# erhant/halo2-vectordb

Measured on AMD Instinct MI355X. Metric: constraints/sec, proving hot path (witness+layout+commit MSM+NTT), kmeans k=16 circuit, higher is better.
Workload: dtype u32x8 (BN254 Fr/Fq, 254-bit Montgomery)

## Files before the change

### halo2_vectordb_amd/_lib.py

```python
import ctypes
import os
import subprocess

_HERE = os.path.dirname(os.path.abspath(__file__))
LIB_PATH = os.path.join(_HERE, "libvdb_hip.so")
CSRC = os.path.join(_HERE, "csrc")


class VdbError(RuntimeError):
    def __init__(self, code, msg):
        super().__init__(f"vdb error {code}: {msg}")
        self.code = code


def build(force=False, jobs=8):
    cmd = ["make", "-C", CSRC, f"-j{jobs}"]
    if force:
        cmd.append("-B")
    subprocess.check_call(cmd)
    return LIB_PATH


_lib = None

# ... 51 lines not shown
    "vdb_ann_index_apply_dev": [_P, _P, _P, _P, _P, _SZ, _SZ, _SZ, _U32, _P, _P, _P, _P, _SZ, _P, _P, _P, _P, _P],
    "vdb_wit_ann_delete_size": [_SZ, _SZ, _SZ, _SZ, _P, _P, _P, _P, _P],
    "vdb_wit_ann_delete": [_P, _P, _SZ, _SZ, _SZ, _SZ, _P, _SZ, _P, _P, _P],
    "vdb_wit_ann_delete_dev": [_P, _P, _SZ, _SZ, _SZ, _SZ, _P, _SZ, _P, _P, _P],
    "vdb_ann_index_remove_size": [_P, _SZ, _SZ, _P, _SZ, _P, _P, _P],
    "vdb_ann_index_remove_dev": [_P, _P, _P, _P, _SZ, _SZ, _SZ, _P, _P, _SZ, _P, _P, _P, _P, _P],
    "vdb_wit_ann_audit_size": [_I, _U32, _U32, _SZ, _SZ, _SZ, _P, _P, _P],
    "vdb_wit_ann_audit": [_I, _U32, _U32, _P, _P, _P, _SZ, _SZ, _SZ, _SZ, _P, _P, _P, _P, _P],
    "vdb_wit_ann_audit_dev": [_I, _U32, _U32, _P, _P, _P, _P, _P, _SZ, _SZ, _SZ, _SZ, _P, _P, _P, _P, _P],
    "vdb_wit_ann_mean_size": [_U32, _U32, _SZ, _SZ, _SZ, _P, _P, _P],
    "vdb_wit_ann_mean": [_U32, _U32, _P, _P, _P, _SZ, _SZ, _SZ, _SZ, _P, _P, _P, _P, _P],
    "vdb_wit_ann_mean_dev": [_U32, _U32, _P, _P, _P, _P, _P, _SZ, _SZ, _SZ, _SZ, _P, _P, _P, _P, _P],
    "vdb_ann_cluster_means_dev": [_U32, _U32, _P, _P, _SZ, _SZ, _SZ, _P],
    "vdb_ann_cluster_means": [_U32, _U32, _P, _P, _SZ, _SZ, _SZ, _P],
    "vdb_wit_nearest_batch_size": [_I, _U32, _U32, _SZ, _SZ, _SZ, _P, _P],
    "vdb_wit_nearest_batch": [_I, _U32, _U32, _P, _P, _SZ, _SZ, _SZ, _P, _P, _P, _P, _P],
    "vdb_wit_nearest_batch_dev": [_I, _U32, _U32, _P, _P, _SZ, _SZ, _SZ, _P, _P, _P, _P, _P],
    "vdb_wit_nearest_topk_size": [_I, _U32, _U32, _SZ, _SZ, _SZ, _SZ, _P, _P],
    "vdb_wit_nearest_topk": [_I, _U32, _U32, _P, _P, _SZ, _SZ, _SZ, _SZ, _P, _P, _P, _P, _P],
    "vdb_wit_nearest_topk_dev": [_I, _U32, _U32, _P, _P, _SZ, _SZ, _SZ, _SZ, _P, _P, _P, _P, _P],
    "vdb_nearest_values": [_U32, _U32, _I, _P, _P, _SZ, _SZ, _SZ, _P, _P],
    "vdb_nearest_values_dev": [_U32, _U32, _I, _P, _P, _SZ, _SZ, _SZ, _P, _P],
    "vdb_layout_plan": [_P, _U64, _U32, _U32, _P, _U64, _P], "vdb_layout_plan_dev": [_P, _U64, _U32, _U32, _P, _U64, _P],
    "vdb_layout_columns": [_P, _U64, _P, _U64, _P, _U64, _U32, _U32, _P, _P, _U64],
    "vdb_layout_columns_dev": [_P, _U64, _P, _U64, _U32, _P, _P, _U32],
    "vdb_layout_lookup_dev": [_P, _U64, _U32, _U32, _P, _U64, _P, _U32],
    "vdb_layout_columns_range_dev": [_P, _U64, _P, _U64, _U32, _U64, _U64, _P, _P, _U32],
    "vdb_layout_lookup_range_dev": [_P, _U64, _U32, _U32, _U64, _U64, _P, _P, _U32], "vdb_wit_set_window": [_U64, _U64, _U64, _U64],
    "vdb_g1_sum": [_P, _SZ, _SZ, _P], "vdb_srs_load": [_U32, _P, _P, _P], "vdb_srs_load_window": [_U32, _P, _P, _U32, _P], "vdb_srs_setup_unsafe": [_U32, _P, _P, _P], "vdb_srs_free": [_P], "vdb_srs_info": [_P, _P, _P, _P],
    "vdb_msm": [_P, _I, _P, _SZ, _P], "vdb_msm_batch": [_P, _I, _P, _SZ, _SZ, _P], "vdb_msm_batch_dev": [_P, _I, _P, _SZ, _SZ, _P],
    "vdb_msm_batch_masked_dev": [_P, _I, _P, _SZ, _SZ, _P, _P, _P], "vdb_layout_const_mask_dev": [_P, _U64, _P, _U64, _U32, _P],
    "vdb_mask_select_dev": [_P, _P, _U64, _I, _P],
    "vdb_msm_count_entries_dev": [_P, _P, _SZ, _SZ, _P, _P],
    "vdb_msm_batch_masked_dev_begin": [_P, _I, _P, _SZ, _SZ, _P, _P], "vdb_msm_batch_end": [_P, _SZ],
    "vdb_grand_product_dev": [_P, _P, _SZ, _SZ, _P], "vdb_eval_polys_dev": [_P, _SZ, _SZ, _P, _P], "vdb_extended_to_coeff_dev": [_P, _SZ, _U32, _U32],
    "vdb_gate_eval_dev": [_P, _P, _SZ, _U32, _U32, _P, _P], "vdb_permutation_mapping_pack_dev": [_P, _SZ, _U32, _P], "vdb_permutation_sigma_packed_dev": [_P, _SZ, _SZ, _U32, _P, _P],
    "vdb_eval_polys_dev_out": [_P, _SZ, _SZ, _P, _P], "vdb_transcript_flush": [_P],
    "vdb_gate_eval_sub_dev": [_P, _U32, _P, _SZ, _U32, _U32, _P, _P], "vdb_divide_by_vanishing_dev": [_P, _U32, _U32],
    "vdb_layout_selectors_dev": [_P, _U64, _P, _U64, _U32, _P],
    "vdb_lookup_permute_dev": [_P, _P, _SZ, _SZ, _SZ, _U32, _P, _P],
    "vdb_lookup_product_dev": [_P, _P, _P, _P, _SZ, _SZ, _SZ, _P, _P, _P], "vdb_fr_delta": [_P],
    "vdb_permutation_sigma_dev": [_P, _SZ, _U32, _P, _P],
    "vdb_transcript_new": [_U32, _U32, _U32, _P], "vdb_transcript_free": [_P], "vdb_transcript_set_sign_bit": [_P, _U32], "vdb_transcript_common_scalar": [_P, _P], "vdb_transcript_common_point": [_P, _P],
    "vdb_transcript_write_points": [_P, _P, _SZ], "vdb_transcript_write_scalars": [_P, _P, _SZ], "vdb_transcript_common_points": [_P, _P, _SZ], "vdb_transcript_common_scalars": [_P, _P, _SZ],
    "vdb_transcript_write_scalar": [_P, _P], "vdb_transcript_write_point": [_P, _P], "vdb_transcript_squeeze": [_P, _P],
    "vdb_transcript_proof_len": [_P, _P], "vdb_transcript_proof_bytes": [_P, _P, _SZ],
    "vdb_scratch_release": [], "vdb_mem_info": [_P, _P], "vdb_scratch_held": [_P], "vdb_msm_set_scratch_cap": [_SZ], "vdb_alloc_stats": [_P, _P, _P, _I],
    "vdb_permutation_mapping_dev": [_P, _U64, _U64, _P, _U64, _U32, _P, _U64, _U64, _U64, _P, _U64, _P],
    "vdb_permutation_mapping_ws_dev": [_P, _U64, _U64, _P, _U64, _U32, _P, _U64, _U64, _U64, _P, _U64, _P, _P, _SZ],
    "vdb_gather_fr_dev": [_P, _P, _SZ, _P], "vdb_copymap_init_dev": [_U64, _U64, _P, _P, _P, _P],
    "vdb_copymap_place_dev": [_P, _P, _P, _U64, _P, _U64, _P, _P, _P, _U64, _U64, _U64, _U64, _P, _P, _P, _P],
    "vdb_copymap_finish_dev": [_P, _P, _U64, _P, _U64, _P, _P, _P], "vdb_mock_check_instances_dev": [_P, _U64, _P, _P, _U64, _P],
    "vdb_fill_rows_dev": [_P, _SZ, _SZ, _SZ, _P],
    "vdb_poly_axpy_dev": [_P, _P, _P, _SZ], "vdb_poly_scale_dev": [_P, _P, _SZ],
    "vdb_poly_lincomb_dev": [_P, _SZ, _SZ, _P, _P], "vdb_kate_div_dev": [_P, _SZ, _SZ, _P, _P, _P],
    "vdb_permutation_eval_dev": [_P, _P, _P, _SZ, _SZ, _U32, _U32, _SZ, _P, _P, _P, _P, _P, _P, _P, _P],
    "vdb_permutation_eval_range_dev": [_P, _P, _P, _SZ, _SZ, _U32, _U32, _SZ, _P, _P, _P, _P, _P, _P, _P, _P, _SZ, _SZ],
    "vdb_coeff_to_cosets_dev": [_P, _P, _SZ, _U32, _U32, _P], "vdb_cosets_to_coeff_dev": [_P, _P, _U32, _U32],
    "vdb_gate_eval_cosets_dev": [_P, _U32, _P, _SZ, _U32, _U32, _P, _P],
    "vdb_lookup_eval_cosets_dev": [_P, _P, _P, _P, _P, _SZ, _U32, _U32, _P, _P, _P, _P, _P, _P, _P],
    "vdb_permutation_eval_parts_cosets_dev": [_P, _SZ, _P, _P, _SZ, _P, _P, _SZ, _SZ, _U32, _U32, _SZ, _P, _P, _P, _P, _P, _P, _P, _P, _I, _SZ, _SZ, _SZ, _SZ],
    "vdb_lookup_eval_dev": [_P, _P, _P, _P, _P, _SZ, _U32, _U32, _P, _P, _P, _P, _P, _P, _P],
    "vdb_permutation_product_dev": [_P, _P, _SZ, _U32, _SZ, _SZ, _P, _P, _P, _P],
    "vdb_permutation_product_range_dev": [_P, _P, _SZ, _SZ, _U32, _SZ, _SZ, _P, _P, _P, _P], "vdb_permutation_chain_dev": [_P, _SZ, _U32, _SZ],
    "vdb_permutation_eval_parts_dev": [_P, _SZ, _P, _P, _SZ, _P, _P, _SZ, _SZ, _U32, _U32, _SZ, _P, _P, _P, _P, _P, _P, _P, _P, _I, _SZ, _SZ, _SZ, _SZ],
    "vdb_colsrc_build_dev": [_P, _U64, _P, _U64, _U32, _U64, _U64, _P, _U32, _P],
# ... 46 lines not shown
```

### halo2_vectordb_amd/csrc/msm.hip

```cpp
#include "common.hpp"
#include "ec.hpp"
#include "ec_l9.hpp"
#include "limb9.hpp"

struct vdb_srs {
  uint32_t k;
  size_t n;
  uint32_t c, W, B;
  vdb::Affine* table[2];
  int device;
};
#define VDB_SRS_HERE(srs) VDB_ARG((srs)->device == vdb::ctx().device, "this srs handle was loaded on another device (vdb_set_device)")

namespace vdb {

#define MSM_SORT_THREADS 1024
#define MSM_LCAP_MIN 32
#define MSM_LCAP_MAX 256

struct MsmRange {
  uint32_t col, bucket, start, len, seg0, pad;
};
struct MsmSegInfo {
  uint32_t idx, len;
};

__global__ __launch_bounds__(256) void k_srs_table(const Affine* __restrict__ bases, Affine* __restrict__ table, size_t n, uint32_t c, uint32_t W) {
  size_t i = (size_t)blockIdx.x * blockDim.x + threadIdx.x;
  if (i >= n) return;
  Affine p = ld_affine(bases + i);
  const u256 m32 = to_mont<Fq>(u256_from_u64(32));
  for (uint32_t j = 0; j < W; j++) {
    Affine ps;
    ps.x = fq_mul(p.x, m32);
    ps.y = fq_mul(p.y, m32);
    st_affine(table + (size_t)j * n + i, ps);
// ... 419 lines not shown
    for (uint32_t q = 0; q < rg.len; q++) {
      const uint32_t pos = rg.start + q;
      if (pos == next) {
        flush_l9(raw + (size_t)seg * (MSM_RAW_WORDS / 4), acc, ident);
        {
          const uint32_t s0 = so[b];
          seginfo[seg].idx = seg - s0;
          seginfo[seg].len = so[b + 1] - s0;
        }
        seg++;
        ident = true;
        do {
          b++;
          next = bo[b + 1];
        } while (next == pos);
      }
      Affine p = nxt;
      bool neg = (v >> 31) != 0;
      if (q + 1 < rg.len) {
        v = e[pos + 1];
        nxt = ld_affine(table + (v & 0x7fffffffu));
      }
      if (!affine_is_identity(p)) madd_l9(acc, ident, p, neg, K);
    }
    flush_l9(raw + (size_t)seg * (MSM_RAW_WORDS / 4), acc, ident);
    {
      const uint32_t s0 = so[b];
      seginfo[seg].idx = seg - s0;
      seginfo[seg].len = so[b + 1] - s0;
    }
  }
}

__global__ __launch_bounds__(256) void k_msm_combine(uint4* __restrict__ raw, const MsmSegInfo* __restrict__ seginfo, const uint32_t* __restrict__ counters,
                                                     uint32_t pass, uint32_t task_cap, MsmL9Consts K) {
  if (counters[1]) return;
  if ((1u << pass) >= counters[2]) return;
  const uint32_t total = counters[0] < task_cap ? counters[0] : task_cap;
  const uint32_t stride = gridDim.x * blockDim.x;
  for (uint32_t t = blockIdx.x * blockDim.x + threadIdx.x; t < total; t += stride) {
    const MsmSegInfo si = seginfo[t];
    const uint32_t len = (si.len + (1u << pass) - 1) >> pass, half = (len + 1) >> 1;
    if (len <= 1 || si.idx + half >= len) continue;
    AccL9 a, b;
    bool a_id, b_id;
    ld_raw_l9(raw + (size_t)t * (MSM_RAW_WORDS / 4), a, a_id);
    ld_raw_l9(raw + (size_t)(t + half) * (MSM_RAW_WORDS / 4), b, b_id);
    xyzz_add_l9(a, a_id, b, b_id, K);
    flush_l9(raw + (size_t)t * (MSM_RAW_WORDS / 4), a, a_id);
  }
}

__device__ __forceinline__ L9 shfl_l9(const L9& v, int src) {
  L9 r;
#pragma unroll
  for (int i = 0; i < 9; i++) r.l[i] = (uint32_t)__shfl((int)v.l[i], src, 64);
  return r;
}
__device__ __forceinline__ AccL9 shfl_acc_l9(const AccL9& p, int src) {
  AccL9 r;
  r.x = shfl_l9(p.x, src);
  r.y = shfl_l9(p.y, src);
  r.zz = shfl_l9(p.zz, src);
  r.zzz = shfl_l9(p.zzz, src);
  return r;
}
__device__ __forceinline__ AccL9 acc_l9_zero() {
  AccL9 r;
#pragma unroll
  for (int i = 0; i < 9; i++) r.x.l[i] = r.y.l[i] = r.zz.l[i] = r.zzz.l[i] = 0;
  return r;
}

__global__ __launch_bounds__(64) void k_msm_reduce(const uint4* __restrict__ raw, const uint32_t* __restrict__ task_off, uint32_t c,
                                                   const uint32_t* __restrict__ counters, const Affine* __restrict__ add_points, uint4* __restrict__ sums,
                                                   MsmL9Consts K) {
// ... 73 lines not shown
  gen.y = to_mont<Fq>(u256_from_u64(2));
  u256 e = u256_from_u64(i);
  u256 ti = mont_pow<Fr>(tau, e), wi = mont_pow<Fr>(omega, e);
  u256 li = fr_mul(fr_mul(wi, tn_minus_1_over_n), mont_inv<Fr>(fr_sub(tau, wi)));
  for (int which = 0; which < 2; which++) {
    u256 k = from_mont<Fr>(which == 0 ? ti : li);
    XYZZ acc = xyzz_identity();
    for (int b = (int)u256_bits(k) - 1; b >= 0; b--) {
      acc = xyzz_double(acc);
      if (u256_bit(k, (unsigned)b)) xyzz_add_mixed(acc, gen, false);
    }
    st_affine((which == 0 ? g : gl) + i, xyzz_to_affine(acc));
  }
}

__global__ __launch_bounds__(64) void k_g1_sum(const Affine* __restrict__ parts, uint32_t m, uint64_t n, Affine* __restrict__ out) {
  const uint64_t c = (uint64_t)blockIdx.x * blockDim.x + threadIdx.x;
  if (c >= n) return;
  XYZZ acc = xyzz_identity();
  for (uint32_t i = 0; i < m; i++) xyzz_add_mixed(acc, ld_affine(parts + (uint64_t)i * n + c), false);
  st_affine(out + c, xyzz_to_affine(acc));
}

static uint32_t pick_window(uint32_t k) {
  const char* env = getenv("VDB_MSM_C");
  if (env) {
    int v = atoi(env);
    if (v >= 2 && v <= 14) return (uint32_t)v;
  }
  if (k <= 8) return 8;
  return 11;
}

int msm_batch_dev(const vdb_srs* srs, int basis, const u256* scalars_dev, size_t n_cols, size_t n, Affine* out_dev, const uint8_t* skip_mask = nullptr,
                  const Affine* add_points = nullptr, bool defer_tail = false, const ColSrc* srcs = nullptr, uint32_t n_blind = 0) {
  Context& cx = ctx();
  if (g_prof_mode == 1) defer_tail = false;
  if (cx.msm_pending) {
    set_error("msm: a deferred batch has not been collected (vdb_msm_batch_end)");
    return VDB_ERR_ARG;
  }
  if (n_cols == 0) return VDB_OK;
  const Affine* table = srs->table[basis];
  const uint32_t c = srs->c, W = srs->W, B = srs->B;
  const size_t ent_cap = n * W;
  uint32_t lcap = MSM_LCAP_MIN;
  while (lcap < MSM_LCAP_MAX && (n_cols * n) / lcap >= ((size_t)1 << 19)) lcap <<= 1;
  const size_t range_cap_col = (ent_cap + lcap - 1) / lcap;
  const size_t seg_cap_col = B + range_cap_col;
  size_t per_col = ent_cap * 4 + range_cap_col * sizeof(MsmRange) + seg_cap_col * (sizeof(MsmSegInfo) + MSM_RAW_WORDS * 4) + MSM_RAW_WORDS * 4 + 2 * (B + 1) * 4 +
                   n * 12;
  static const bool two_phase_on = !(getenv("VDB_MSM_TWO_PHASE") && getenv("VDB_MSM_TWO_PHASE")[0] == '0');
  uint32_t idx_bits = 1;
  while (((uint64_t)1 << idx_bits) < (uint64_t)W * srs->n) idx_bits++;
  uint32_t fine_bits = 0;
  const uint32_t bin_cap = MSM_BIN_CAP;
  if (two_phase_on && c >= 13) {
    fine_bits = c - 1 - 8;
    if (fine_bits + idx_bits > 31) fine_bits = idx_bits < 31 ? 31 - idx_bits : 0;
    if (fine_bits < 2) fine_bits = 0;
  }
  size_t free_b = 0, total_b = 0;
  if (hipMemGetInfo(&free_b, &total_b) != hipSuccess) free_b = (size_t)80 << 30;
  size_t budget = (free_b + cx.scratch_bytes[2]) / 2;
  if (budget < ((size_t)8 << 30)) budget = (size_t)8 << 30;
  if (budget > ((size_t)96 << 30)) budget = (size_t)96 << 30;
  if (cx.msm_scratch_cap && budget > cx.msm_scratch_cap) budget = cx.msm_scratch_cap > cx.scratch_bytes[2] ? cx.msm_scratch_cap : cx.scratch_bytes[2];
  size_t nb = budget / per_col;
  if (nb < 1) nb = 1;
  if (nb > n_cols) nb = n_cols;
  if (nb > 16384) nb = 16384;
  if (nb * seg_cap_col > 0x7fffffffull) nb = 0x7fffffffull / seg_cap_col;
  uint8_t* buf = (uint8_t*)scratch_get(2, nb * per_col + 512);
  if (!buf) return VDB_ERR_OOM;
  uint32_t* entries = (uint32_t*)buf;
  uint4* raw = (uint4*)(buf + nb * ent_cap * 4);
  uint4* sums = (uint4*)((uint8_t*)raw + nb * seg_cap_col * MSM_RAW_WORDS * 4);
  MsmRange* ranges = (MsmRange*)((uint8_t*)sums + nb * MSM_RAW_WORDS * 4);
  MsmSegInfo* seginfo = (MsmSegInfo*)((uint8_t*)ranges + nb * range_cap_col * sizeof(MsmRange));
  uint32_t* seg_off = (uint32_t*)((uint8_t*)seginfo + nb * seg_cap_col * sizeof(MsmSegInfo));
  uint32_t* bucket_off = seg_off + nb * (B + 1);
  uint32_t* counters = bucket_off + nb * (B + 1);
  unsigned long long* recs = (unsigned long long*)(((uintptr_t)(counters + 64) + 7) & ~(uintptr_t)7);
  uint32_t* longq = (uint32_t*)(recs + nb * n);
  const uint32_t seg_cap = (uint32_t)(nb * seg_cap_col), range_cap = (uint32_t)(nb * range_cap_col);
  size_t lds = (3 * (size_t)B + 32) * sizeof(uint32_t);
  MsmL9Consts l9k;
  l9_offset_limbs<FqParams>(2, l9k.c2);
  l9_offset_limbs<FqParams>(8, l9k.c8);
  l9k.one_rp = to_mont<Fq>(u256_from_u64(32));
  l9k.to_std = mont_one<Fq>();
  l9k.to_rp = to_mont<Fq>(u256_from_u64(1024));
  for (size_t c0 = 0; c0 < n_cols; c0 += nb) {
    size_t nc = n_cols - c0 < nb ? n_cols - c0 : nb;
    if (c0 == 0) {
      VDB_HIP(hipMemsetAsync(counters, 0, 4 * sizeof(uint32_t), cx.stream));
    } else {
      VDB_HIP(hipMemsetAsync(counters, 0, sizeof(uint32_t), cx.stream));
      VDB_HIP(hipMemsetAsync(counters + 2, 0, 2 * sizeof(uint32_t), cx.stream));
    }
    {
      VDB_PROF("k_msm_sort");
      hipLaunchKernelGGL(k_msm_sort, dim3((unsigned)nc), dim3(MSM_SORT_THREADS), lds, cx.stream, scalars_dev ? scalars_dev + c0 * n : nullptr, srcs ? srcs + c0 : nullptr,
                       n_blind, n, srs->n, c, W, entries,
                       ent_cap, seg_off, bucket_off, ranges, counters, seg_cap, range_cap, skip_mask ? skip_mask + c0 * n : nullptr,
                       lcap, longq, recs, fine_bits, idx_bits, bin_cap);
    }
    VDB_LAUNCH_CHECK();
    if (fine_bits) {
      VDB_PROF("k_msm_scatter2");
      const unsigned bins_x = (B >> fine_bits) < 64u ? (B >> fine_bits) : 64u;
      hipLaunchKernelGGL(k_msm_scatter2, dim3(bins_x, (unsigned)nc), dim3(MSM_SCATTER2_THREADS), (bin_cap + (1u << fine_bits)) * sizeof(uint32_t), cx.stream,
                       entries, ent_cap, bucket_off, B, fine_bits, idx_bits, bin_cap, counters);
    }
    VDB_LAUNCH_CHECK();
    {
      VDB_PROF("k_msm_accum");
      hipLaunchKernelGGL(k_msm_accum, dim3((unsigned)(cx.cu_count * 8)), dim3(256), 0, cx.stream, table, entries, ent_cap, ranges, bucket_off, B,
                       seg_off, counters, raw, seginfo, range_cap, l9k);
    }
    VDB_LAUNCH_CHECK();
    hipStream_t ts = cx.stream;
    if (defer_tail && c0 + nc == n_cols) {
      VDB_HIP(hipEventRecord(cx.ev_tail, cx.stream));
      VDB_HIP(hipStreamWaitEvent(cx.aux, cx.ev_tail, 0));
      ts = cx.aux;
    }
    {
      uint32_t max_nt = (uint32_t)range_cap_col + 1, passes = 0;
      while ((1u << passes) < max_nt) passes++;
      for (uint32_t ps = 0; ps < passes; ps++) {
        VDB_PROF_ON("k_msm_combine", ts);
        hipLaunchKernelGGL(k_msm_combine, dim3((unsigned)(cx.cu_count * 8)), dim3(256), 0, ts, raw, seginfo, counters, ps, seg_cap, l9k);
      }
      VDB_LAUNCH_CHECK();
    }
    {
      VDB_PROF_ON("k_msm_reduce", ts);
      hipLaunchKernelGGL(k_msm_reduce, dim3((unsigned)nc), dim3(64), 0, ts, raw, seg_off, c, counters, add_points ? add_points + c0 : nullptr, sums, l9k);
    }
    VDB_LAUNCH_CHECK();
    {
      VDB_PROF_ON("k_msm_normalise", ts);
      hipLaunchKernelGGL(k_msm_normalise, dim3((unsigned)((nc + 63) / 64)), dim3(64), 0, ts, sums, (uint32_t)nc, counters, l9k.to_std, out_dev + c0);
    }
    VDB_LAUNCH_CHECK();
  }
  if (defer_tail) {
    cx.msm_pending = true;
    cx.msm_counters = counters;
    return VDB_OK;
  }
  uint32_t h_counters[2] = {0, 0};
  VDB_HIP(hipMemcpyAsync(h_counters, counters, sizeof(h_counters), hipMemcpyDeviceToHost, cx.stream));
  VDB_HIP(hipStreamSynchronize(cx.stream));
  if (h_counters[1]) {
    set_error("msm: internal task buffer overflow");
    return VDB_ERR_HIP;
  }
  return VDB_OK;
}

int msm_collect() {
  Context& cx = ctx();
  if (!cx.msm_pending) return VDB_OK;
  cx.msm_pending = false;
// ... 141 lines not shown
int vdb_msm_batch_dev(const vdb_srs* srs, int basis, const vdb_fr* scalars_dev, size_t n_cols, size_t n, vdb_g1* out_host) {
  VDB_REQUIRE_INIT();
  VDB_ARG(srs && scalars_dev && out_host && (basis == 0 || basis == 1), "bad argument");
  VDB_SRS_HERE(srs);
  VDB_ARG(srs->table[basis], "srs was loaded without this basis");
  VDB_ARG(n <= srs->n && n > 0, "n exceeds the loaded SRS size (shorter columns are allowed)");
  if (n_cols == 0) return VDB_OK;
  Affine* dout = (Affine*)scratch_get(1, n_cols * sizeof(Affine));
  if (!dout) return VDB_ERR_OOM;
  int rc = msm_batch_dev(srs, basis, as_u256(scalars_dev), n_cols, n, dout);
  if (rc) return rc;
  VDB_HIP(hipMemcpyAsync(out_host, dout, n_cols * sizeof(Affine), hipMemcpyDeviceToHost, ctx().stream));
  VDB_HIP(hipStreamSynchronize(ctx().stream));
  return VDB_OK;
}
int vdb_msm_count_entries_dev(const vdb_srs* srs, const vdb_fr* scalars_dev, size_t n_cols, size_t n, const uint8_t* skip_mask_dev, uint64_t* counts_out) {
  VDB_REQUIRE_INIT();
  VDB_ARG(srs && scalars_dev && counts_out && n <= srs->n, "bad argument");
  VDB_SRS_HERE(srs);
  if (n_cols == 0) return VDB_OK;
  Context& cx = ctx();
  unsigned long long* d = (unsigned long long*)scratch_get(2, n_cols * sizeof(unsigned long long));
  if (!d) return VDB_ERR_OOM;
  VDB_HIP(hipMemsetAsync(d, 0, n_cols * sizeof(unsigned long long), cx.stream));
  {
    VDB_PROF("k_msm_count_entries");
    hipLaunchKernelGGL(k_msm_count_entries, dim3((unsigned)n_cols), dim3(256), 0, cx.stream, as_u256(scalars_dev), skip_mask_dev, (uint64_t)n, srs->c, srs->W, d);
  }
  VDB_LAUNCH_CHECK();
  VDB_HIP(hipMemcpyAsync(counts_out, d, n_cols * sizeof(uint64_t), hipMemcpyDeviceToHost, cx.stream));
  VDB_HIP(hipStreamSynchronize(cx.stream));
  return VDB_OK;
}
int vdb_msm_batch_masked_dev_begin(const vdb_srs* srs, int basis, const vdb_fr* scalars_dev, size_t n_cols, size_t n, const uint8_t* skip_mask_dev,
                                   const vdb_g1* const_points_dev) {
  VDB_REQUIRE_INIT();
  VDB_ARG(srs && scalars_dev && (basis == 0 || basis == 1), "bad argument");
  VDB_SRS_HERE(srs);
  VDB_ARG(srs->table[basis], "srs was loaded without this basis");
  VDB_ARG(n <= srs->n && n > 0, "n exceeds the loaded SRS size");
  VDB_ARG((skip_mask_dev == nullptr) == (const_points_dev == nullptr), "mask and constant points go together");
  if (n_cols == 0) return VDB_OK;
  VDB_ARG(!ctx().msm_pending, "msm: a deferred batch has not been collected (vdb_msm_batch_end)");
  Affine* dout = (Affine*)deferred_out(n_cols * sizeof(Affine));
  if (!dout) return VDB_ERR_OOM;
  ctx().msm_out = dout;
  int rc = msm_batch_dev(srs, basis, as_u256(scalars_dev), n_cols, n, dout, skip_mask_dev, reinterpret_cast<const Affine*>(const_points_dev), true);
  if (rc == VDB_OK && !ctx().msm_pending) ctx().msm_pending = true;
  return rc;
}
int vdb_msm_batch_src_dev_begin(const vdb_srs* srs, int basis, const vdb_colsrc* src_dev, size_t n_cols, size_t n, uint32_t n_blind,
                                const uint8_t* skip_mask_dev, const vdb_g1* const_points_dev) {
  VDB_REQUIRE_INIT();
  VDB_ARG(srs && src_dev && (basis == 0 || basis == 1), "bad argument");
  VDB_SRS_HERE(srs);
  VDB_ARG(srs->table[basis], "srs was loaded without this basis");
  VDB_ARG(n <= srs->n && n > 0 && n_blind <= n, "n exceeds the loaded SRS size");
  VDB_ARG((skip_mask_dev == nullptr) == (const_points_dev == nullptr), "mask and constant points go together");
  if (n_cols == 0) return VDB_OK;
  VDB_ARG(!ctx().msm_pending, "msm: a deferred batch has not been collected (vdb_msm_batch_end)");
  Affine* dout = (Affine*)deferred_out(n_cols * sizeof(Affine));
  if (!dout) return VDB_ERR_OOM;
  ctx().msm_out = dout;
  int rc = msm_batch_dev(srs, basis, nullptr, n_cols, n, dout, skip_mask_dev, reinterpret_cast<const Affine*>(const_points_dev), true,
                         reinterpret_cast<const ColSrc*>(src_dev), n_blind);
  if (rc == VDB_OK && !ctx().msm_pending) ctx().msm_pending = true;
// ... 46 lines not shown
```

### include/vdb.h

```cpp
#ifndef VDB_H
#define VDB_H
#include <stddef.h>
#include <stdint.h>

#ifdef __cplusplus
extern "C" {
#endif

typedef struct { uint64_t l[4]; } vdb_fr;
typedef struct { uint64_t l[4]; } vdb_fq;
typedef struct { vdb_fq x, y; } vdb_g1;
typedef struct { vdb_fq x[2], y[2]; } vdb_g2;
typedef struct vdb_srs vdb_srs;

enum {
  VDB_OK = 0,
  VDB_ERR_NOT_INIT = -1,
  VDB_ERR_HIP = -2,
  VDB_ERR_ARG = -3,
  VDB_ERR_OOM = -4,
  VDB_ERR_DOMAIN = -5,
  VDB_ERR_NO_DEVICE = -6
};

// ... 195 lines not shown
                         uint64_t col_hi, const vdb_fr *blind_dev, uint32_t n_blind, vdb_colsrc *out_dev);
int vdb_colsrc_build_lookup_dev(const vdb_fr *lookup_dev, uint64_t n_cells, uint32_t k, uint32_t minimum_rows, uint64_t col_lo, uint64_t col_hi,
                                const vdb_fr *blind_dev, uint32_t n_blind, vdb_colsrc *out_dev);
int vdb_layout_columns_range_dev(const vdb_fr *stream_dev, uint64_t n_cells, const uint64_t *break_points, uint64_t n_bp, uint32_t k, uint64_t col_lo,
                                 uint64_t col_hi, vdb_fr *cols_dev, const vdb_fr *blind_dev, uint32_t n_blind);
int vdb_layout_lookup_range_dev(const vdb_fr *lookup_dev, uint64_t n_cells, uint32_t k, uint32_t minimum_rows, uint64_t col_lo, uint64_t col_hi,
                                vdb_fr *cols_dev, const vdb_fr *blind_dev, uint32_t n_blind);
int vdb_layout_const_mask_dev(const uint8_t *flags_dev, uint64_t n_cells, const uint64_t *break_points, uint64_t n_bp, uint32_t k, uint8_t *mask_dev);
int vdb_mask_select_dev(const vdb_fr *in_dev, const uint8_t *mask_dev, uint64_t n, int keep_const, vdb_fr *out_dev);

int vdb_srs_load(uint32_t k, const vdb_g1 *g, const vdb_g1 *g_lagrange, vdb_srs **out);
int vdb_srs_load_window(uint32_t k, const vdb_g1 *g, const vdb_g1 *g_lagrange, uint32_t window_bits, vdb_srs **out);
int vdb_srs_setup_unsafe(uint32_t k, const vdb_fr *tau, vdb_g1 *g_out, vdb_g1 *g_lagrange_out);
int vdb_g1_check_dev(const vdb_g1 *pts_dev, size_t n, uint64_t *n_bad, uint64_t *first_bad);
int vdb_g1_lagrange_from_monomial_dev(uint32_t k, const vdb_g1 *g_dev, vdb_g1 *g_lagrange_dev);
int vdb_srs_downsize(uint32_t k, const vdb_g1 *g_host, vdb_g1 *g_lagrange_out);
void vdb_srs_free(vdb_srs *srs);
int vdb_g1_sum(const vdb_g1 *parts, size_t m, size_t n, vdb_g1 *out);
int vdb_srs_device(const vdb_srs *srs, int *device);
int vdb_srs_info(const vdb_srs *srs, uint32_t *k, uint32_t *window_bits, uint32_t *windows);

int vdb_msm(const vdb_srs *srs, int basis, const vdb_fr *scalars, size_t n, vdb_g1 *out);
int vdb_msm_batch(const vdb_srs *srs, int basis, const vdb_fr *const *cols, size_t n_cols, size_t n, vdb_g1 *out);
int vdb_srs_load_all(uint32_t k, const vdb_g1 *g, const vdb_g1 *g_lagrange, uint32_t window_bits, vdb_srs **out, int n_out);
int vdb_msm_batch_multi(vdb_srs *const *srs, int n_srs, int basis, const vdb_fr *const *cols, size_t n_cols, size_t n, vdb_g1 *out);
int vdb_msm_batch_dev(const vdb_srs *srs, int basis, const vdb_fr *scalars_dev, size_t n_cols, size_t n, vdb_g1 *out_host);
int vdb_msm_batch_masked_dev_begin(const vdb_srs *srs, int basis, const vdb_fr *scalars_dev, size_t n_cols, size_t n, const uint8_t *skip_mask_dev,
                                   const vdb_g1 *const_points_dev);
int vdb_msm_batch_src_dev_begin(const vdb_srs *srs, int basis, const vdb_colsrc *src_dev, size_t n_cols, size_t n, uint32_t n_blind,
                                const uint8_t *skip_mask_dev, const vdb_g1 *const_points_dev);
int vdb_msm_batch_end(vdb_g1 *out_host, size_t n_cols);
int vdb_msm_count_entries_dev(const vdb_srs *srs, const vdb_fr *scalars_dev, size_t n_cols, size_t n, const uint8_t *skip_mask_dev,
                              uint64_t *counts_out);
int vdb_msm_batch_masked_dev(const vdb_srs *srs, int basis, const vdb_fr *scalars_dev, size_t n_cols, size_t n, const uint8_t *skip_mask_dev,
                             const vdb_g1 *const_points_dev, vdb_g1 *out_host);

#define VDB_NTT_INVERSE_SCALE 1
int vdb_ntt_batch(vdb_fr *const *cols, size_t n_cols, uint32_t log_n, const vdb_fr *omega, int flags);
int vdb_ntt_batch_multi(vdb_fr *const *cols, size_t n_cols, uint32_t log_n, const vdb_fr *omega, int flags);
int vdb_ntt_batch_dev(vdb_fr *cols_dev, size_t n_cols, uint32_t log_n, const vdb_fr *omega, int flags);
int vdb_lagrange_to_coeff(vdb_fr *const *cols, size_t n_cols, uint32_t k);
int vdb_lagrange_to_coeff_dev(vdb_fr *cols_dev, size_t n_cols, uint32_t k);
int vdb_lagrange_to_coeff_src_dev(const vdb_colsrc *src_dev, vdb_fr *coeff_dev, size_t n_cols, uint32_t k, uint32_t n_blind);
int vdb_grand_product_dev(const vdb_fr *num_dev, const vdb_fr *den_dev, size_t n_cols, size_t n, vdb_fr *z_dev);
int vdb_eval_polys_dev(const vdb_fr *coeff_dev, size_t n_cols, size_t n, const vdb_fr *x, vdb_fr *out_host);
int vdb_eval_polys_dev_out(const vdb_fr *coeff_dev, size_t n_cols, size_t n, const vdb_fr *x, vdb_fr *out_dev);
int vdb_lookup_permute_dev(const vdb_fr *input_dev, const vdb_fr *table_dev, size_t n_cols, size_t n, size_t usable_rows, uint32_t max_bits,
                           vdb_fr *permuted_input_dev, vdb_fr *permuted_table_dev);
int vdb_lookup_product_dev(const vdb_fr *input_dev, const vdb_fr *table_dev, const vdb_fr *perm_input_dev, const vdb_fr *perm_table_dev, size_t n_cols, size_t n,
                           size_t usable_rows, const vdb_fr *beta, const vdb_fr *gamma, vdb_fr *z_dev);
int vdb_fr_delta(vdb_fr *out);
int vdb_permutation_sigma_dev(const uint64_t *mapping_dev, size_t n_cols, uint32_t k, const vdb_fr *delta, vdb_fr *sigma_dev);
int vdb_permutation_mapping_pack_dev(const uint64_t *mapping_dev, size_t n_cols, uint32_t k, uint32_t *packed_dev);
int vdb_permutation_sigma_packed_dev(const uint32_t *packed_block_dev, size_t n_block_cols, size_t n_cols_total, uint32_t k, const vdb_fr *delta,
                                     vdb_fr *sigma_block_dev);
int vdb_permutation_product_dev(const vdb_fr *cols_dev, const vdb_fr *sigma_dev, size_t n_cols, uint32_t k, size_t usable_rows, size_t chunk_len,
                                const vdb_fr *beta, const vdb_fr *gamma, const vdb_fr *delta, vdb_fr *z_dev);
int vdb_permutation_eval_dev(const vdb_fr *adv_ext_dev, const vdb_fr *sigma_ext_dev, const vdb_fr *z_ext_dev, size_t n_cols, size_t chunk_len, uint32_t k,
                             uint32_t ext_k, size_t usable_rows, const vdb_fr *l0_ext_dev, const vdb_fr *l_last_ext_dev, const vdb_fr *l_active_ext_dev,
                             const vdb_fr *beta, const vdb_fr *gamma, const vdb_fr *delta, const vdb_fr *y, vdb_fr *acc_dev);
int vdb_permutation_eval_range_dev(const vdb_fr *adv_ext_dev, const vdb_fr *sigma_ext_block_dev, const vdb_fr *z_ext_dev, size_t n_cols, size_t chunk_len,
                                   uint32_t k, uint32_t ext_k, size_t usable_rows, const vdb_fr *l0_ext_dev, const vdb_fr *l_last_ext_dev,
                                   const vdb_fr *l_active_ext_dev, const vdb_fr *beta, const vdb_fr *gamma, const vdb_fr *delta, const vdb_fr *y, vdb_fr *acc_dev,
                                   size_t set_lo, size_t set_hi);
int vdb_permutation_product_range_dev(const vdb_fr *cols_block_dev, const vdb_fr *sigma_block_dev, size_t n_block_cols, size_t col0, uint32_t k,
                                      size_t usable_rows, size_t chunk_len, const vdb_fr *beta, const vdb_fr *gamma, const vdb_fr *delta, vdb_fr *z_block_dev);
// ... 99 lines not shown
```

Before: 1.979 billion.

## Compact MSM segment-combine passes via per-pass worklists built by a plan kernel

Adds a planning kernel that, after bucket accumulation, computes for each tree-reduction pass which segments actually perform an add and writes compacted index lists using ballot/popcount and atomics. The combine kernel then iterates only over its pass's list instead of scanning all segments each pass. The goal is to cut idle thread scans and divergence across the log-many combine launches, at the cost of an extra kernel, extra scratch memory for the lists, and a larger counter memset. It also adds host-side debug entry points for inspecting the fold rule and plan.

```diff
diff --git a/halo2_vectordb_amd/_lib.py b/halo2_vectordb_amd/_lib.py
--- a/halo2_vectordb_amd/_lib.py
+++ b/halo2_vectordb_amd/_lib.py
@@ -107,6 +107,7 @@
     "vdb_msm_batch_masked_dev": [_P, _I, _P, _SZ, _SZ, _P, _P, _P], "vdb_layout_const_mask_dev": [_P, _U64, _P, _U64, _U32, _P],
     "vdb_mask_select_dev": [_P, _P, _U64, _I, _P],
     "vdb_msm_count_entries_dev": [_P, _P, _SZ, _SZ, _P, _P],
+    "vdb_msm_fold_rule": [_U32, _U32, _U32, _P, _P], "vdb_msm_fold_plan_last": [_U32, _P, _SZ, _P, _P, _SZ, _P],
     "vdb_msm_batch_masked_dev_begin": [_P, _I, _P, _SZ, _SZ, _P, _P], "vdb_msm_batch_end": [_P, _SZ],
     "vdb_grand_product_dev": [_P, _P, _SZ, _SZ, _P], "vdb_eval_polys_dev": [_P, _SZ, _SZ, _P, _P], "vdb_extended_to_coeff_dev": [_P, _SZ, _U32, _U32],
     "vdb_gate_eval_dev": [_P, _P, _SZ, _U32, _U32, _P, _P], "vdb_permutation_mapping_pack_dev": [_P, _SZ, _U32, _P], "vdb_permutation_sigma_packed_dev": [_P, _SZ, _SZ, _U32, _P, _P],
diff --git a/halo2_vectordb_amd/csrc/msm.hip b/halo2_vectordb_amd/csrc/msm.hip
--- a/halo2_vectordb_amd/csrc/msm.hip
+++ b/halo2_vectordb_amd/csrc/msm.hip
@@ -2,6 +2,7 @@
 #include "ec.hpp"
 #include "ec_l9.hpp"
 #include "limb9.hpp"
+#include "msm_fold.hpp"
 
 struct vdb_srs {
   uint32_t k;
@@ -487,16 +488,104 @@
   }
 }
 
+#define MSM_FOLD_COUNTS 8
+#define MSM_FOLD_MAX_PASSES 32
+#define MSM_COUNTER_WORDS 64
+static_assert(MSM_FOLD_COUNTS + MSM_FOLD_MAX_PASSES <= MSM_COUNTER_WORDS, "the per-pass counts lie inside the counter block");
+__host__ __device__ inline uint32_t msm_fold_list_off(uint32_t list_cap, uint32_t pass) {
+  uint32_t off = 0;
+  for (uint32_t q = 0; q < pass; q++) off += list_cap >> q;
+  return off;
+}
+
+#define MSM_PLAN_THREADS 256
+#define MSM_PLAN_PER_THREAD 4
+#define MSM_PLAN_SLOTS (MSM_PLAN_PER_THREAD * MSM_PLAN_THREADS / 64)
+__global__ __launch_bounds__(MSM_PLAN_THREADS) void k_msm_fold_plan(const MsmSegInfo* __restrict__ seginfo, uint32_t* __restrict__ counters,
+                                                                    uint32_t* __restrict__ lists, uint32_t task_cap, uint32_t list_cap) {
+  if (counters[1]) return;
+  const uint32_t max_segs = counters[2];
+  uint32_t np = 0;
+  while (np < MSM_FOLD_MAX_PASSES - 1 && (1u << np) < max_segs) np++;
+  if (np == 0) return;
+  const uint32_t total = counters[0] < task_cap ? counters[0] : task_cap;
+  __shared__ uint32_t s_cnt[MSM_FOLD_MAX_PASSES][MSM_PLAN_SLOTS];
+  __shared__ uint32_t s_base[MSM_FOLD_MAX_PASSES];
+  const uint32_t tid = threadIdx.x, lane = tid & 63, wave = tid >> 6;
+  const unsigned long long below = (1ull << lane) - 1ull;
+  const uint32_t tile = MSM_PLAN_THREADS * MSM_PLAN_PER_THREAD;
+  for (uint32_t t0 = blockIdx.x * tile; t0 < total; t0 += gridDim.x * tile) {
+    MsmSegInfo si[MSM_PLAN_PER_THREAD];
+#pragma unroll
+    for (uint32_t j = 0; j < MSM_PLAN_PER_THREAD; j++) {
+      const uint32_t t = t0 + j * MSM_PLAN_THREADS + tid;
+      si[j].idx = 0;
+      si[j].len = 1;
+      if (t < total) si[j] = seginfo[t];
+    }
+    uint32_t longest = 1, wnp = 0;
+#pragma unroll
+    for (uint32_t j = 0; j < MSM_PLAN_PER_THREAD; j++) longest = si[j].len > longest ? si[j].len : longest;
+    while (wnp < np && __any(longest > (1u << wnp))) wnp++;
+    for (uint32_t p = 0; p < np; p++) {
+#pragma unroll
+      for (uint32_t j = 0; j < MSM_PLAN_PER_THREAD; j++) {
+        uint32_t half, n_add = 0;
+        if (p < wnp) n_add = (uint32_t)__popcll(__ballot(msm_fold_pair(si[j].idx, si[j].len, p, &half)));
+        if (lane == 0) s_cnt[p][j * (MSM_PLAN_THREADS / 64) + wave] = n_add;
+      }
+    }
+    __syncthreads();
+    if (tid < np) {
+      uint32_t sum = 0;
+      for (uint32_t s = 0; s < MSM_PLAN_SLOTS; s++) {
+        const uint32_t v = s_cnt[tid][s];
+        s_cnt[tid][s] = sum;
+        sum += v;
+      }
+      uint32_t base = 0xffffffffu;
+      if (sum) {
+        const uint32_t cap = list_cap >> tid;
+        base = atomicAdd(&counters[MSM_FOLD_COUNTS + tid], sum);
+        if (base > cap || sum > cap - base) {
+          atomicExch(&counters[1], 1u);
+          base = 0xffffffffu;
+        } else {
+          base += msm_fold_list_off(list_cap, tid);
+        }
+      }
+      s_base[tid] = base;
+    }
+    __syncthreads();
+    for (uint32_t p = 0; p < wnp; p++) {
+      const uint32_t base = s_base[p];
+      if (base == 0xffffffffu) continue;
+#pragma unroll
+      for (uint32_t j = 0; j < MSM_PLAN_PER_THREAD; j++) {
+        uint32_t half;
+        const bool adds = msm_fold_pair(si[j].idx, si[j].len, p, &half);
+        const unsigned long long m = __ballot(adds);
+        if (adds) lists[base + s_cnt[p][j * (MSM_PLAN_THREADS / 64) + wave] + (uint32_t)__popcll(m & below)] = t0 + j * MSM_PLAN_THREADS + tid;
+      }
+    }
+    __syncthreads();
+  }
+}
+
 __global__ __launch_bounds__(256) void k_msm_combine(uint4* __restrict__ raw, const MsmSegInfo* __restrict__ seginfo, const uint32_t* __restrict__ counters,
-                                                     uint32_t pass, uint32_t task_cap, MsmL9Consts K) {
+                                                     const uint32_t* __restrict__ lists, uint32_t pass, uint32_t task_cap, uint32_t list_cap, MsmL9Consts K) {
   if (counters[1]) return;
-  if ((1u << pass) >= counters[2]) return;
-  const uint32_t total = counters[0] < task_cap ? counters[0] : task_cap;
+  const uint32_t cap = list_cap >> pass;
+  const uint32_t count = counters[MSM_FOLD_COUNTS + pass] < cap ? counters[MSM_FOLD_COUNTS + pass] : cap;
+  if (count == 0) return;
+  const uint32_t* list = lists + msm_fold_list_off(list_cap, pass);
   const uint32_t stride = gridDim.x * blockDim.x;
-  for (uint32_t t = blockIdx.x * blockDim.x + threadIdx.x; t < total; t += stride) {
+  for (uint32_t i = blockIdx.x * blockDim.x + threadIdx.x; i < count; i += stride) {
+    const uint32_t t = list[i];
+    if (t >= task_cap) continue;
     const MsmSegInfo si = seginfo[t];
-    const uint32_t len = (si.len + (1u << pass) - 1) >> pass, half = (len + 1) >> 1;
-    if (len <= 1 || si.idx + half >= len) continue;
+    uint32_t half;
+    if (!msm_fold_pair(si.idx, si.len, pass, &half)) continue;
     AccL9 a, b;
     bool a_id, b_id;
     ld_raw_l9(raw + (size_t)t * (MSM_RAW_WORDS / 4), a, a_id);
@@ -636,6 +725,17 @@
   return 11;
 }
 
+struct MsmFoldPlanView {
+  const void* buf = nullptr;
+  size_t bytes = 0;
+  const uint32_t* counters = nullptr;
+  const uint32_t* lists = nullptr;
+  const MsmSegInfo* seginfo = nullptr;
+  uint32_t seg_cap = 0, list_cap = 0;
+  int device = -1;
+};
+static MsmFoldPlanView g_fold_plan_view;
+
 int msm_batch_dev(const vdb_srs* srs, int basis, const u256* scalars_dev, size_t n_cols, size_t n, Affine* out_dev, const uint8_t* skip_mask = nullptr,
                   const Affine* add_points = nullptr, bool defer_tail = false, const ColSrc* srcs = nullptr, uint32_t n_blind = 0) {
   Context& cx = ctx();
@@ -652,8 +752,8 @@
   while (lcap < MSM_LCAP_MAX && (n_cols * n) / lcap >= ((size_t)1 << 19)) lcap <<= 1;
   const size_t range_cap_col = (ent_cap + lcap - 1) / lcap;
   const size_t seg_cap_col = B + range_cap_col;
-  size_t per_col = ent_cap * 4 + range_cap_col * sizeof(MsmRange) + seg_cap_col * (sizeof(MsmSegInfo) + MSM_RAW_WORDS * 4) + MSM_RAW_WORDS * 4 + 2 * (B + 1) * 4 +
-                   n * 12;
+  size_t per_col = ent_cap * 4 + range_cap_col * (sizeof(MsmRange) + 2 * 4) + seg_cap_col * (sizeof(MsmSegInfo) + MSM_RAW_WORDS * 4) + MSM_RAW_WORDS * 4 +
+                   2 * (B + 1) * 4 + n * 12;
   static const bool two_phase_on = !(getenv("VDB_MSM_TWO_PHASE") && getenv("VDB_MSM_TWO_PHASE")[0] == '0');
   uint32_t idx_bits = 1;
   while (((uint64_t)1 << idx_bits) < (uint64_t)W * srs->n) idx_bits++;
@@ -682,13 +782,22 @@
   uint4* sums = (uint4*)((uint8_t*)raw + nb * seg_cap_col * MSM_RAW_WORDS * 4);
   MsmRange* ranges = (MsmRange*)((uint8_t*)sums + nb * MSM_RAW_WORDS * 4);
   MsmSegInfo* seginfo = (MsmSegInfo*)((uint8_t*)ranges + nb * range_cap_col * sizeof(MsmRange));
-  uint32_t* seg_off = (uint32_t*)((uint8_t*)seginfo + nb * seg_cap_col * sizeof(MsmSegInfo));
+  uint32_t* fold_lists = (uint32_t*)((uint8_t*)seginfo + nb * seg_cap_col * sizeof(MsmSegInfo));
+  uint32_t* seg_off = fold_lists + 2 * nb * range_cap_col;
   uint32_t* bucket_off = seg_off + nb * (B + 1);
   uint32_t* counters = bucket_off + nb * (B + 1);
-  unsigned long long* recs = (unsigned long long*)(((uintptr_t)(counters + 64) + 7) & ~(uintptr_t)7);
+  unsigned long long* recs = (unsigned long long*)(((uintptr_t)(counters + MSM_COUNTER_WORDS) + 7) & ~(uintptr_t)7);
   uint32_t* longq = (uint32_t*)(recs + nb * n);
   const uint32_t seg_cap = (uint32_t)(nb * seg_cap_col), range_cap = (uint32_t)(nb * range_cap_col);
   size_t lds = (3 * (size_t)B + 32) * sizeof(uint32_t);
+  g_fold_plan_view.buf = buf;
+  g_fold_plan_view.bytes = nb * per_col + 512;
+  g_fold_plan_view.counters = counters;
+  g_fold_plan_view.lists = fold_lists;
+  g_fold_plan_view.seginfo = seginfo;
+  g_fold_plan_view.seg_cap = seg_cap;
+  g_fold_plan_view.list_cap = range_cap;
+  g_fold_plan_view.device = cx.device;
   MsmL9Consts l9k;
   l9_offset_limbs<FqParams>(2, l9k.c2);
   l9_offset_limbs<FqParams>(8, l9k.c8);
@@ -698,10 +807,10 @@
   for (size_t c0 = 0; c0 < n_cols; c0 += nb) {
     size_t nc = n_cols - c0 < nb ? n_cols - c0 : nb;
     if (c0 == 0) {
-      VDB_HIP(hipMemsetAsync(counters, 0, 4 * sizeof(uint32_t), cx.stream));
+      VDB_HIP(hipMemsetAsync(counters, 0, MSM_COUNTER_WORDS * sizeof(uint32_t), cx.stream));
     } else {
       VDB_HIP(hipMemsetAsync(counters, 0, sizeof(uint32_t), cx.stream));
-      VDB_HIP(hipMemsetAsync(counters + 2, 0, 2 * sizeof(uint32_t), cx.stream));
+      VDB_HIP(hipMemsetAsync(counters + 2, 0, (MSM_COUNTER_WORDS - 2) * sizeof(uint32_t), cx.stream));
     }
     {
       VDB_PROF("k_msm_sort");
@@ -731,11 +840,16 @@
       ts = cx.aux;
     }
     {
+      VDB_PROF_ON("k_msm_fold_plan", ts);
+      hipLaunchKernelGGL(k_msm_fold_plan, dim3((unsigned)(cx.cu_count * 8)), dim3(MSM_PLAN_THREADS), 0, ts, seginfo, counters, fold_lists, seg_cap, range_cap);
+    }
+    VDB_LAUNCH_CHECK();
+    {
       uint32_t max_nt = (uint32_t)range_cap_col + 1, passes = 0;
       while ((1u << passes) < max_nt) passes++;
       for (uint32_t ps = 0; ps < passes; ps++) {
         VDB_PROF_ON("k_msm_combine", ts);
-        hipLaunchKernelGGL(k_msm_combine, dim3((unsigned)(cx.cu_count * 8)), dim3(256), 0, ts, raw, seginfo, counters, ps, seg_cap, l9k);
+        hipLaunchKernelGGL(k_msm_combine, dim3((unsigned)(cx.cu_count * 8)), dim3(256), 0, ts, raw, seginfo, counters, fold_lists, ps, seg_cap, range_cap, l9k);
       }
       VDB_LAUNCH_CHECK();
     }
@@ -943,6 +1057,38 @@
   VDB_HIP(hipStreamSynchronize(cx.stream));
   return VDB_OK;
 }
+int vdb_msm_fold_rule(uint32_t idx, uint32_t len, uint32_t pass, uint32_t* adds, uint32_t* half) {
+  VDB_ARG(adds && half && len >= 1 && idx < len, "bad argument");
+  *half = 0;
+  *adds = msm_fold_pair(idx, len, pass, half) ? 1u : 0u;
+  return VDB_OK;
+}
+int vdb_msm_fold_plan_last(uint32_t pass, uint32_t* list_out, size_t list_room, uint32_t* count_out, uint32_t* seginfo_out, size_t seg_room,
+                           uint32_t* segments_out) {
+  VDB_REQUIRE_INIT();
+  VDB_ARG(count_out && segments_out && pass < MSM_FOLD_MAX_PASSES, "bad argument");
+  Context& cx = ctx();
+  const MsmFoldPlanView& v = g_fold_plan_view;
+  VDB_ARG(!cx.msm_pending, "msm: a deferred batch has not been collected (vdb_msm_batch_end)");
+  VDB_ARG(v.buf && v.device == cx.device && v.buf == cx.scratch[2] && cx.scratch_bytes[2] >= v.bytes, "no MSM work space of this device holds a folding plan");
+  VDB_HIP(hipStreamSynchronize(cx.aux));
+  VDB_HIP(hipStreamSynchronize(cx.stream));
+  uint32_t h[MSM_COUNTER_WORDS];
+  VDB_HIP(hipMemcpy(h, v.counters, sizeof(h), hipMemcpyDeviceToHost));
+  const uint32_t segments = h[0] < v.seg_cap ? h[0] : v.seg_cap, cap = v.list_cap >> pass;
+  const uint32_t count = h[MSM_FOLD_COUNTS + pass] < cap ? h[MSM_FOLD_COUNTS + pass] : cap;
+  *count_out = count;
+  *segments_out = segments;
+  if (list_out) {
+    VDB_ARG(list_room >= count, "list_out is too small");
+    if (count) VDB_HIP(hipMemcpy(list_out, v.lists + msm_fold_list_off(v.list_cap, pass), (size_t)count * 4, hipMemcpyDeviceToHost));
+  }
+  if (seginfo_out) {
+    VDB_ARG(seg_room >= segments, "seginfo_out is too small");
+    if (segments) VDB_HIP(hipMemcpy(seginfo_out, v.seginfo, (size_t)segments * sizeof(MsmSegInfo), hipMemcpyDeviceToHost));
+  }
+  return VDB_OK;
+}
 int vdb_msm_batch_masked_dev_begin(const vdb_srs* srs, int basis, const vdb_fr* scalars_dev, size_t n_cols, size_t n, const uint8_t* skip_mask_dev,
                                    const vdb_g1* const_points_dev) {
   VDB_REQUIRE_INIT();
diff --git a/halo2_vectordb_amd/csrc/msm_fold.hpp b/halo2_vectordb_amd/csrc/msm_fold.hpp
--- /dev/null
+++ b/halo2_vectordb_amd/csrc/msm_fold.hpp
@@ -0,0 +1,14 @@
+#pragma once
+#include <hip/hip_runtime.h>
+#include <stdint.h>
+
+namespace vdb {
+
+__host__ __device__ inline bool msm_fold_pair(uint32_t idx, uint32_t len, uint32_t pass, uint32_t* half) {
+  if (pass >= 31) return false;
+  const uint32_t len_p = (len + (1u << pass) - 1) >> pass;
+  *half = (len_p + 1) >> 1;
+  return len_p > 1 && idx < (len_p >> 1);
+}
+
+}
diff --git a/include/vdb.h b/include/vdb.h
--- a/include/vdb.h
+++ b/include/vdb.h
@@ -251,6 +251,9 @@
 int vdb_msm_batch_end(vdb_g1 *out_host, size_t n_cols);
 int vdb_msm_count_entries_dev(const vdb_srs *srs, const vdb_fr *scalars_dev, size_t n_cols, size_t n, const uint8_t *skip_mask_dev,
                               uint64_t *counts_out);
+int vdb_msm_fold_rule(uint32_t idx, uint32_t len, uint32_t pass, uint32_t *adds, uint32_t *half);
+int vdb_msm_fold_plan_last(uint32_t pass, uint32_t *list_out, size_t list_room, uint32_t *count_out, uint32_t *seginfo_out, size_t seg_room,
+                           uint32_t *segments_out);
 int vdb_msm_batch_masked_dev(const vdb_srs *srs, int basis, const vdb_fr *scalars_dev, size_t n_cols, size_t n, const uint8_t *skip_mask_dev,
                              const vdb_g1 *const_points_dev, vdb_g1 *out_host);
 
```

New measurement: 1.989 billion (median of 6 runs). No clear change (+0.5%).
